# meenzen/Stl.Fusion

Hardware: AMD Instinct MI355X
Metric: invalidated nodes/sec + GTEPS at 1/2/4/8 MI355X; achieved HBM GB/s vs peak (higher is better)
Workload: dtype u64

## Files before the change

### include/fgi.h

```cpp
#ifndef FGI_H
#define FGI_H
#include <stddef.h>
#include <stdint.h>

#ifdef __cplusplus
extern "C" {
#endif

typedef int fgi_status;
#define FGI_OK 0
#define FGI_EINVAL 1
#define FGI_ENOMEM 2
#define FGI_ECAPACITY 3
#define FGI_EDEVICE 4
#define FGI_ESTATE 5
#define FGI_ENOTSUP 6

#define FGI_NONE 0xFFFFFFFFu

#define FGI_COMPUTING 0u
#define FGI_CONSISTENT 1u
#define FGI_INVALIDATED 2u
#define FGI_STATE_MASK 3u
#define FGI_F_INVALIDATE_ON_SET_OUTPUT 4u
// ... 158 lines not shown
fgi_status fgi_stream(fgi_graph* g, void** stream);
#define FGI_OPT_DEAD_FILTER 1
#define FGI_OPT_DIRECTION 2
#define FGI_OPT_PULL_ALPHA 3
#define FGI_OPT_LEVEL_TIMING 4
#define FGI_OPT_PULL_BETA 5
#define FGI_OPT_DEFRAG_PCT 6
#define FGI_OPT_PART_COLLECTIVES 7
#define FGI_OPT_PULL_TPB 8
#define FGI_OPT_FRONT_EXCHANGE 9
#define FGI_OPT_HOT_HEADS 10
#define FGI_OPT_FAULT_INJECT 11
#define FGI_OPT_PART_PLAN 13
#define FGI_OPT_PART_BUCKET 14
#define FGI_OPT_FAULT_INJECT_TAIL 16
fgi_status fgi_set_option(fgi_graph* g, int option, int64_t value);

fgi_status fgi_part_unique_id(uint8_t* id128);
fgi_status fgi_part_init(fgi_graph* g, uint32_t n_global, const uint8_t* id128);
typedef int (*fgi_allgather_fn)(void* ctx, const void* send, uint64_t bytes, void* recv);
fgi_status fgi_part_init_host(fgi_graph* g, uint32_t n_global, fgi_allgather_fn fn, void* ctx);
fgi_status fgi_part_synth_rmat(fgi_graph* g, uint32_t scale, uint32_t edge_factor, uint64_t seed,
                               uint32_t stale_pct, uint64_t stale_seed);
fgi_status fgi_part_register_nodes(fgi_graph* g, uint32_t n, const uint32_t* slot, const uint64_t* version,
                                   const uint32_t* state_flags);
fgi_status fgi_part_load_edges(fgi_graph* g, uint64_t m, const uint32_t* used, const uint32_t* dependant,
                               const uint64_t* tag);
fgi_status fgi_part_invalidate(fgi_graph* g, uint32_t n_roots, const uint32_t* roots_dev,
                               const uint8_t* immediately_dev, uint64_t* out_n, fgi_wave_stats* stats);
fgi_status fgi_part_export_ids(fgi_graph* g, uint32_t* out_ids, uint64_t cap, uint64_t* out_n);
// ... 27 lines not shown
```

### stl.fusion_amd/csrc/fgi_internal.h

```cpp
#pragma once
#include <hip/hip_runtime.h>
#include <stdint.h>

#include <chrono>
#include <cstdlib>
#include <string>
#include <utility>
#include <vector>

#include "../../include/fgi.h"
#include "../../include/fgi_variants.h"

#ifndef FGI_VARIANTS
#define FGI_VARIANTS 0
#endif

namespace fgi {

constexpr uint64_t kVMask = (1ull << 56) - 1;
constexpr int kStateShift = 56;
constexpr uint64_t kStateBits = 3ull << kStateShift;
constexpr uint64_t kW_IOSO = 1ull << 58;
constexpr uint64_t kW_DS = 1ull << 59;
constexpr uint64_t kW_HasDelay = 1ull << 60;
// ... 70 lines not shown
    *src = rmat_scramble(s, scale, seed);
    *dst = rmat_scramble(d, scale, seed);
}
__host__ __device__ inline bool synth_stale(uint32_t stale_pct, uint64_t stale_seed, uint32_t src, uint32_t dst) {
    return stale_pct && (sm64(stale_seed ^ sm64(((uint64_t)src << 32) | dst)) % 100) < stale_pct;
}

constexpr int kRing = 64;
constexpr int kBlock = 256;
constexpr int kEPT = 8;
constexpr int kChunk = kBlock * kEPT;
constexpr int kFine = 256;
constexpr uint32_t kStatBlocks = 8192;
constexpr int kStatCols = 8;
constexpr int kPullTile = 1024;
constexpr int kDoneGroups = 16;
constexpr int kDoneStride = 16;
#ifndef FGI_FINAL_BLOCKS
#define FGI_FINAL_BLOCKS 1024
#endif
#ifndef FGI_FINAL_WPB
#define FGI_FINAL_WPB 256
#endif
#ifndef FGI_INIT_BLOCKS
#define FGI_INIT_BLOCKS 2048
#endif
constexpr uint32_t kFinalBlocks = FGI_FINAL_BLOCKS;
constexpr uint32_t kFinalWpb = FGI_FINAL_WPB;
constexpr uint32_t kInitBlocks = FGI_INIT_BLOCKS;
#ifndef FGI_SPIN_WAIT
// ... 246 lines not shown
    std::vector<uint32_t> flg_drop;
    uint32_t* inv_bm = nullptr;
    uint64_t bm_words = 0;

    uint64_t* uin_off = nullptr;
    uint32_t* uin_len = nullptr;
    uint32_t* uin_src = nullptr;
    uint64_t* uin_head = nullptr;
    uint32_t* uin_more = nullptr;
    uint64_t uin_cap = 0;
    unsigned long long* pool_live = nullptr;
    uint64_t pool_live_cap = 0;
    uint64_t pl_mut_epoch = 0, pl_pool_epoch = ~0ull;
    uint4* cand = nullptr;
    uint32_t* cand_seg = nullptr;
    uint32_t* wl = nullptr;
    uint32_t* hot_id = nullptr;
    uint32_t n_hot = 0;
    uint64_t hot_w0 = 0;
    uint4* sv[2] = {nullptr, nullptr};
    uint32_t* sv_cnt[2] = {nullptr, nullptr};
    uint64_t cand_cap = 0;
    uint32_t cand_grid = 0;
    uint64_t uin_epoch = 0;
    uint64_t mut_epoch = 1;
    uint64_t epoch_counter = 1;
    uint64_t snap_mut_epoch = 0;

    int opt_dead_filter = 1;
    int opt_defrag_pct = 60;
    int opt_part_coll = 0;
    int opt_front_exchange = 0;
    uint64_t stale_est = 0;
    uint32_t prune_cursor = 0;
    int opt_direction = 0;
    int opt_pull_alpha = 28;
    int opt_pull_tpb = 0;
    int opt_hot_heads = 0;
    uint32_t* sum_bm = nullptr;
    int64_t opt_sum_min = -1;
    int opt_pull_beta = 32;
    int opt_level_timing = 1;
    int opt_fused = fgi::fused_default();

    void* scratch = nullptr;
    size_t scratch_bytes = 0;
    unsigned long long* misc_dev = nullptr;
    unsigned long long* misc_host = nullptr;

    uint64_t* snap_node = nullptr;
    uint64_t* snap_row_off = nullptr;
    uint32_t* snap_row_len = nullptr;
    uint32_t* snap_row_cap = nullptr;
// ... 184 lines not shown
```

### stl.fusion_amd/csrc/graph.hip

```cpp
#include <hip/hip_runtime.h>
#include <hip/hip_cooperative_groups.h>

#include <rocprim/device/device_radix_sort.hpp>
#include <rocprim/device/device_reduce.hpp>
#include <rocprim/device/device_segmented_radix_sort.hpp>
#include <rocprim/device/device_scan.hpp>

#include <algorithm>
#include <cstddef>
#include <chrono>
#include <cstdarg>
#include <cstdio>
#include <cstring>

#include "fgi_internal.h"

namespace fgi {

fgi_status set_err(fgi_graph* g, fgi_status st, const char* fmt, ...) {
    if (g) {
        char buf[512];
        va_list ap;
        va_start(ap, fmt);
        vsnprintf(buf, sizeof(buf), fmt, ap);
// ... 1056 lines not shown
    const uint64_t key = k < k_max ? sorted[k] : 0ull;
    if ((key >> 32) == 0) {
        hot_id[k] = FGI_NONE;
        return;
    }
    hot_id[k] = (uint32_t)key;
    hot_rank[(uint32_t)key] = k;
}

__device__ __forceinline__ uint32_t head_code(uint32_t h, const uint32_t* hot_rank, uint32_t hot_bit0) {
    if (h == FGI_NONE || !hot_rank) return h;
    const uint32_t r = hot_rank[h];
    return r != FGI_NONE ? (hot_bit0 + r) : h;
}

__global__ void k_cand_fill(uint32_t n, const uint32_t* __restrict__ flag, const uint32_t* __restrict__ pos,
                            const uint64_t* __restrict__ uin_head, const uint32_t* __restrict__ uin_len,
                            const uint32_t* __restrict__ row_len, const uint32_t* __restrict__ hot_rank,
                            uint32_t hot_bit0, uint4* cand, unsigned long long* too_long) {
    const uint32_t d = blockIdx.x * blockDim.x + threadIdx.x;
    if (d >= n || !flag[d]) return;
    const uint32_t p = pos[d], rl = row_len[d];
    if (rl >> 31) atomicAdd(too_long, 1ull);
    const uint64_t h = uin_head[d];
    cand[p] = make_uint4(d, (rl & 0x7FFFFFFFu) | (uin_len[d] > 2 ? 0x80000000u : 0u),
                         head_code((uint32_t)h, hot_rank, hot_bit0), head_code((uint32_t)(h >> 32), hot_rank, hot_bit0));
}

__global__ void k_cand_seg(uint32_t G, uint64_t span, uint32_t n, const uint32_t* __restrict__ pos, uint32_t total,
                           uint32_t* seg) {
    const uint32_t b = blockIdx.x * blockDim.x + threadIdx.x;
    if (b > G) return;
    const uint64_t s0 = (uint64_t)b * span;
    seg[b] = s0 < n ? pos[s0] : total;
}

__global__ void k_invalidate_all_roots(uint32_t n_slots, const unsigned long long* node, uint32_t* roots,
                                       unsigned long long* cnt) {
    const uint32_t s = blockIdx.x * blockDim.x + threadIdx.x;
    if (s < n_slots && word_is_current(node[s])) roots[atomicAdd(cnt, 1ull)] = s;
}

inline uint32_t nblk(uint64_t n, uint32_t b = 256) { return (uint32_t)((n + b - 1) / b); }

template <class T>
fgi_status h2d(fgi_graph* g, T* dst, const T* src, size_t count) {
    if (count == 0) return FGI_OK;
    FGI_HIP(g, hipMemcpyAsync(dst, src, count * sizeof(T), hipMemcpyHostToDevice, g->stream));
    return FGI_OK;
// ... 226 lines not shown
    if (G == 0) return FGI_OK;
    hipStream_t s = g->stream;
    const uint32_t N = g->n_slots;
    if (g->cand_cap < N || !g->cand) {
        dfree(g->cand);
        dfree(g->wl);
        for (int k = 0; k < 2; ++k) dfree(g->sv[k]);
        g->cand_cap = 0;
        FGI_TRY(dmalloc(g, &g->cand, N));
        FGI_TRY(dmalloc(g, &g->wl, N));
        for (int k = 0; k < 2; ++k) FGI_TRY(dmalloc(g, &g->sv[k], N));
        g->cand_cap = N;
    }
    if (!g->cand_seg) {
        FGI_TRY(dmalloc(g, &g->cand_seg, (size_t)kStatBlocks + 1));
        FGI_TRY(dmalloc(g, &g->sv_cnt[0], kStatBlocks));
        FGI_TRY(dmalloc(g, &g->sv_cnt[1], kStatBlocks));
    }
    Tmp tf, tp, ts;
    uint32_t *flag, *pos;
    FGI_TRY(tmalloc(g, tf, &flag, N));
    FGI_TRY(tmalloc(g, tp, &pos, N));
    hipLaunchKernelGGL(k_cand_flag, dim3(nblk(N)), dim3(256), 0, s, N, g->uin_len, flag);
    size_t tb = 0;
    FGI_HIP(g, rocprim::exclusive_scan(nullptr, tb, flag, pos, 0u, (size_t)N, rocprim::plus<uint32_t>(), s));
    char* tmp;
    FGI_TRY(tmalloc(g, ts, &tmp, tb));
    FGI_HIP(g, rocprim::exclusive_scan(tmp, tb, flag, pos, 0u, (size_t)N, rocprim::plus<uint32_t>(), s));
    uint32_t lp = 0, lf = 0;
    FGI_TRY(d2h(g, &lp, pos + N - 1, 1));
    FGI_TRY(d2h(g, &lf, flag + N - 1, 1));
    const uint32_t total = lp + lf;
    Tmp th;
    uint32_t* hot_rank = nullptr;
    g->n_hot = 0;
    PartView pv;
    const bool part = part_view(g, &pv);
    const uint32_t NH = part ? pv.n_global : g->n_handles;
    g->hot_w0 = part ? pv.front_words_global : g->bm_words;
    if (g->hot_w0 * 32 + kHot < (uint64_t)FGI_NONE) {
        if (!g->hot_id) FGI_TRY(dmalloc(g, &g->hot_id, kHot));
        Tmp tc, tk0, tk1, tt;
        uint32_t* cnt;
        uint64_t *k0, *k1;
        FGI_TRY(tmalloc(g, tc, &cnt, NH));
        FGI_TRY(tmalloc(g, th, &hot_rank, NH));
        FGI_TRY(tmalloc(g, tk0, &k0, NH));
// ... 5 lines not shown
        size_t sb = 0;
        FGI_HIP(g, rocprim::radix_sort_keys_desc(nullptr, sb, k0, k1, (size_t)NH, 0, 64, s));
        char* st;
        FGI_TRY(tmalloc(g, tt, &st, sb));
        FGI_HIP(g, rocprim::radix_sort_keys_desc(st, sb, k0, k1, (size_t)NH, 0, 64, s));
        uint32_t n_hot = hot_count(NH);
        if (g->opt_hot_heads > 0)
            n_hot = std::min<uint32_t>(n_hot, (uint32_t)(g->opt_hot_heads + 255) / 256 * 256);
        hipLaunchKernelGGL(k_hot_pick, dim3(n_hot / 256), dim3(256), 0, s, NH, n_hot, k1, g->hot_id, hot_rank);
        FGI_HIP(g, hipGetLastError());
        FGI_HIP(g, hipStreamSynchronize(s));
        g->n_hot = n_hot;
    }
    FGI_HIP(g, hipMemsetAsync(g->misc_dev + 15, 0, sizeof(unsigned long long), s));
    hipLaunchKernelGGL(k_cand_fill, dim3(nblk(N)), dim3(256), 0, s, N, flag, pos, g->uin_head, g->uin_len, g->row_len,
                       hot_rank, (uint32_t)(g->hot_w0 * 32), g->cand, g->misc_dev + 15);
    hipLaunchKernelGGL(k_cand_seg, dim3(nblk(G + 1)), dim3(256), 0, s, G, (uint64_t)tpb * kPullTile, N, pos, total,
                       g->cand_seg);
    FGI_HIP(g, hipGetLastError());
    unsigned long long too_long = 0;
    FGI_TRY(d2h(g, &too_long, g->misc_dev + 15, 1));
    if (too_long == 0) g->cand_grid = G;
    if (getenv("FGI_TRACE"))
        fprintf(stderr, "[fgi] candidates: %u of %u slots, pull grid %u x %u tiles, %u hot heads, %llu rows too long\n", total,
                N, G, tpb, g->n_hot, (unsigned long long)too_long);
    return FGI_OK;
}

fgi_status build_rows_from_keys(fgi_graph* g, uint64_t m, uint64_t* keys, uint64_t* tags, uint64_t ver_seed,
                                uint32_t stale_pct, uint64_t stale_seed, uint32_t src_base, uint32_t dst_base) {
    hipStream_t s = g->stream;
    const uint32_t H = g->n_handles;
    FGI_HIP(g, hipMemsetAsync(g->row_off, 0, (size_t)H * sizeof(uint64_t), s));
    FGI_HIP(g, hipMemsetAsync(g->row_len, 0, (size_t)H * sizeof(uint32_t), s));
    FGI_HIP(g, hipMemsetAsync(g->row_cap, 0, (size_t)H * sizeof(uint32_t), s));
    FGI_HIP(g, hipMemsetAsync(g->used_cnt, 0, (size_t)H * sizeof(uint32_t), s));
    g->pool_top = 0;
    g->pool_epoch++;
    touch(g);
    if (m == 0) return FGI_OK;
// ... 335 lines not shown
        dfree(g->fr_off[i]);
        dfree(g->fr_len[i]);
    }
    for (int i = 0; i < 2; ++i) {
        dfree(g->escan[i]);
        dfree(g->cstart[i]);
    }
    dfree(g->uin_off);
    dfree(g->uin_len);
    dfree(g->uin_src);
    dfree(g->uin_head);
    dfree(g->pool_live);
    dfree(g->cand);
    dfree(g->wl);
    dfree(g->cand_seg);
    dfree(g->hot_id);
    for (int k = 0; k < 2; ++k) {
        dfree(g->sv[k]);
        dfree(g->sv_cnt[k]);
    }
    dfree(g->vis_bm);
    dfree(g->vis_spare);
    if (g->flg_bm) (void)hipFree(g->flg_bm);
    if (g->flg_cnt) (void)hipFree(g->flg_cnt);
    for (int k = 0; k < 2; ++k)
        if (g->flg_out[k]) (void)hipFree(g->flg_out[k]);
    dfree(g->cls_bm);
    dfree(g->uin_more);
    dfree(g->sum_bm);
    dfree(g->inv_bm);
// ... 425 lines not shown
        return FGI_OK;
    case FGI_OPT_LEVEL_TIMING: g->opt_level_timing = value ? 1 : 0; return FGI_OK;
    case FGI_OPT_PULL_TPB:
        if (value < 0 || value > 32) return set_err(g, FGI_EINVAL, "pull tiles per block must be 0..32");
        g->opt_pull_tpb = (int)value;
        if (!g->part) {
            g->uin_epoch = 0;
        } else if (g->uin_src && g->uin_epoch == g->mut_epoch) {
            hipSetDevice(g->device);
            return build_candidates(g);
        }
        return FGI_OK;
    case FGI_OPT_HOT_HEADS:
        if (value < 0 || value > (int64_t)kHot) return set_err(g, FGI_EINVAL, "hot heads must be 0..%u", kHot);
        g->opt_hot_heads = (int)value;
        if (!g->part) {
            g->uin_epoch = 0;
        } else if (g->uin_src && g->uin_epoch == g->mut_epoch) {
            hipSetDevice(g->device);
            return build_candidates(g);
        }
        return FGI_OK;
    case FGI_OPT_PULL_BETA:
        if (value < 0) return set_err(g, FGI_EINVAL, "beta must be >= 0");
        g->opt_pull_beta = (int)value;
        return FGI_OK;
    case FGI_OPT_PART_PLAN: g->opt_part_plan = value ? 1 : 0; return FGI_OK;
    case FGI_OPT_PART_BUCKET: return part_set_bucket(g, value);
    case FGI_OPT_PROBE_SUMMARY:
        if (value < -1 || value > (int64_t)FGI_NONE) return set_err(g, FGI_EINVAL, "probe summary: -1 or a word count");
// ... 1527 lines not shown
```

### stl.fusion_amd/csrc/wave.hip

```cpp
#include <hip/hip_cooperative_groups.h>
#include <hip/hip_runtime.h>

#include <sched.h>

#include <algorithm>
#include <chrono>
#include <cstdio>
#include <cstring>
#include <cstdlib>
#include <vector>

#include "fgi_internal.h"

#ifndef FGI_PROBE
#define FGI_PROBE 0
#endif

namespace fgi {
namespace {

__device__ __forceinline__ uint32_t lane_id() { return __lane_id(); }
constexpr int kProbeLevelsOff = 1 << 20;

#if FGI_PROBE
// ... 834 lines not shown

struct PullArgs {
    uint32_t n_slots;
    const uint64_t* __restrict__ uin_off;
    const uint32_t* __restrict__ uin_len;
    const uint32_t* __restrict__ uin_src;
    const uint32_t* front_rd;
    const uint32_t* sum;
    uint32_t hot_bit0;
    uint32_t hot_lds;
    uint32_t* inv_bm;
    const uint32_t* __restrict__ cls;
    uint32_t* wl;
    unsigned long long* bsum;
    const uint32_t* __restrict__ cand_seg;
    const uint4* c[3];
    uint4* sv[2];
    uint32_t* sv_cnt[2];
};

constexpr uint32_t kMaxIter = 32;
#ifndef FGI_CPL
#define FGI_CPL 4
#endif
#ifndef FGI_TAIL_CAP
#define FGI_TAIL_CAP kChunk
#endif
constexpr uint32_t kCPL = FGI_CPL;
constexpr uint32_t kTailCap = FGI_TAIL_CAP;
constexpr uint32_t kTileWords = kPullTile / 64;
constexpr uint32_t kOwnWords = 2 * kMaxIter * kTileWords;
constexpr uint32_t kCandBatch = kCPL * kBlock;
constexpr uint32_t kWaveBatch = kCPL * 64;
constexpr uint32_t kWaveTailCap = kTailCap / (kBlock / 64);
constexpr uint32_t kLaneTail = 12;

struct PullLds {
    uint32_t hot[kLdsHot];
    uint32_t vm[kOwnWords];
    uint32_t wm[kOwnWords];
    uint32_t cs[kOwnWords];
    uint32_t sn;
    uint32_t wn;
};

constexpr uint32_t kPushLds = kChunkEmitCap + 8;
constexpr uint32_t kLevelLds =
    std::max<uint32_t>(kPushLds + (sizeof(MsgEmit<true>) + 7) / 8 * 2, kTailCap + 4 + (sizeof(PullLds) + 3) / 4);
static_assert(kTailCap % 4 == 0 && kWaveBatch <= kTailCap / (kBlock / 64), "pull tail queue");

// ... 5 lines not shown
typedef uint32_t u32x4 __attribute__((ext_vector_type(4)));

__device__ __forceinline__ bool sum_zero(const PullArgs& p, uint32_t h) {
    return !((p.sum[h >> 11] >> ((h >> 6) & 31)) & 1u);
}
__device__ __forceinline__ uint32_t head_bits(const PullArgs& p, const PullLds& s, uint32_t h, bool sum) {
    const uint32_t r = (h - p.hot_bit0) >> 5;
    if (r < p.hot_lds) return s.hot[r];
    if (sum && h < p.hot_bit0 && sum_zero(p, h)) return 0u;
    return p.front_rd[h >> 5];
}
__device__ __forceinline__ bool front_bit(const PullArgs& p, uint32_t u, bool sum) {
    return !(sum && sum_zero(p, u)) && bit_of(p.front_rd, u);
}

__device__ __forceinline__ uint4 load_cand(const uint4* p, bool in, uint32_t s_lo) {
    if (!in) return make_uint4(s_lo, 0u, FGI_NONE, FGI_NONE);
    const u32x4 v = __builtin_nontemporal_load(reinterpret_cast<const u32x4*>(p));
    return make_uint4(v.x, v.y, v.z, v.w);
}

__device__ __forceinline__ void pull_hit(const PullArgs& p, PullLds& s, uint64_t s_lo, uint64_t seg, uint32_t d, bool win,
                                         uint32_t aux, WinSum& ws) {
    const uint32_t rel = (uint32_t)(d - s_lo);
    const uint32_t bit = 1u << (d & 31);
    if (win) {
        atomicOr(&s.wm[rel >> 5], bit);
        const uint32_t rl = aux & 0x7FFFFFFFu;
        ++ws.w;
        if (rl) {
            ++ws.e;
            ws.l += rl;
            p.wl[seg + atomicAdd(&s.wn, 1u)] = d;
        }
    } else {
        atomicOr(&s.vm[rel >> 5], bit);
    }
}

__device__ __forceinline__ void pull_tails(const PullArgs& p, const uint4* src, uint4* sv_out, const unsigned long long* node,
                                           uint64_t s_lo, uint64_t seg, uint32_t* q, uint32_t nq, PullLds& s,
                                           uint32_t& flagged, uint32_t& examined, uint32_t& tails, WinSum& ws, bool sum) {
    const uint32_t lane = lane_id();
    uint32_t nlong = 0;
    for (uint32_t r0 = 0; r0 < nq; r0 += 64) {
        const uint32_t e = r0 + lane;
        const bool in = e < nq;
        uint32_t qi = 0, len = 0;
        uint64_t off = 0;
        uint4 c = make_uint4(0u, 0u, 0u, 0u);
        if (in) {
            qi = q[e];
            c = src[seg + qi];
            len = p.uin_len[c.x];
            off = p.uin_off[c.x];
        }
        const uint32_t u2 = (in && len > 2) ? p.uin_src[off + 2] : FGI_NONE;
        const uint32_t u3 = (in && len > 3) ? p.uin_src[off + 3] : FGI_NONE;
        const bool hit = (u2 != FGI_NONE && front_bit(p, u2, sum)) || (u3 != FGI_NONE && front_bit(p, u3, sum));
        examined += (u2 != FGI_NONE ? 1u : 0u) + (u3 != FGI_NONE ? 1u : 0u);
        const bool more = in && !hit && len > 4;
        const unsigned long long mm = __ballot(more);
        if (more) q[nlong + rank_in(mm)] = qi | (len > kLaneTail ? 0x80000000u : 0u);
        nlong += (uint32_t)__popcll(mm);
        if (in && hit) {
            const uint32_t d = c.x, rel = (uint32_t)(d - s_lo);
            const bool win = (s.cs[rel >> 5] >> (d & 31)) & 1u;
            pull_hit(p, s, s_lo, seg, d, win, c.y, ws);
            if (!win) flagged += first_visit(node[d]) == 2 ? 1u : 0u;
        }
        const bool surv = in && !hit && !more;
        const unsigned long long sm = __ballot(surv);
        if (sm) {
            uint32_t sb = 0;
            if (lane == 0) sb = atomicAdd(&s.sn, (uint32_t)__popcll(sm));
            sb = from_lane0(sb);
            if (surv) sv_out[sb + rank_in(sm)] = c;
        }
        tails += in ? 1u : 0u;
    }
    __builtin_amdgcn_wave_barrier();
    uint32_t nl2 = 0;
    for (uint32_t r0 = 0; r0 < nlong; r0 += 64) {
        const uint32_t e = r0 + lane;
        const uint32_t v = e < nlong ? q[e] : 0u;
        const bool in = e < nlong && !(v >> 31);
        const bool lng = e < nlong && (v >> 31);
        const unsigned long long lm = __ballot(lng);
        if (lng) q[nl2 + rank_in(lm)] = v & 0x7FFFFFFFu;
        nl2 += (uint32_t)__popcll(lm);
        uint4 c = make_uint4(0u, 0u, 0u, 0u);
        uint32_t len = 0;
        uint64_t off = 0;
        if (in) {
            c = src[seg + v];
            len = p.uin_len[c.x];
            off = p.uin_off[c.x];
        }
        uint32_t u[kLaneTail - 4];
#pragma unroll
        for (uint32_t k = 0; k < kLaneTail - 4; ++k) u[k] = (in && 4 + k < len) ? p.uin_src[off + 4 + k] : FGI_NONE;
        bool found = false;
#pragma unroll
        for (uint32_t k = 0; k < kLaneTail - 4; ++k)
            if (u[k] != FGI_NONE) {
                found |= front_bit(p, u[k], sum);
                ++examined;
            }
        if (in && found) {
            const uint32_t d = c.x, rel = (uint32_t)(d - s_lo);
            const bool win = (s.cs[rel >> 5] >> (d & 31)) & 1u;
            pull_hit(p, s, s_lo, seg, d, win, c.y, ws);
            if (!win) flagged += first_visit(node[d]) == 2 ? 1u : 0u;
        }
        const bool surv = in && !found;
        const unsigned long long sm = __ballot(surv);
        if (sm) {
            uint32_t sb = 0;
            if (lane == 0) sb = atomicAdd(&s.sn, (uint32_t)__popcll(sm));
            sb = from_lane0(sb);
            if (surv) sv_out[sb + rank_in(sm)] = c;
        }
    }
    nlong = nl2;
    __builtin_amdgcn_wave_barrier();
    const uint32_t sub = lane & 7, grp = lane >> 3;
    constexpr uint32_t G8 = 8;
    uint4 c_n = make_uint4(0u, 0u, 0u, 0u);
    uint32_t len_n = 0;
    uint64_t off_n = 0;
    if (grp < nlong) {
        c_n = src[seg + q[grp]];
        len_n = p.uin_len[c_n.x];
        off_n = p.uin_off[c_n.x];
    }
    for (uint32_t e = grp; e < nlong; e += G8) {
        const uint4 c = c_n;
        const uint32_t len = len_n;
        const uint64_t off = off_n;
        if (e + G8 < nlong) {
            c_n = src[seg + q[e + G8]];
            len_n = p.uin_len[c_n.x];
            off_n = p.uin_off[c_n.x];
        }
        bool found = false;
        for (uint32_t r = 4; r < len && !found; r += 8) {
            const uint32_t k = r + sub;
            const bool x = k < len && front_bit(p, p.uin_src[off + k], sum);
            examined += (k < len) ? 1u : 0u;
            found = ((__ballot(x) >> (lane & ~7u)) & 0xFFull) != 0;
        }
        if (sub == 0) {
            const uint32_t d = c.x;
            if (found) {
                const uint32_t rel = (uint32_t)(d - s_lo);
                const bool win = (s.cs[rel >> 5] >> (d & 31)) & 1u;
                pull_hit(p, s, s_lo, seg, d, win, c.y, ws);
                if (!win) flagged += first_visit(node[d]) == 2 ? 1u : 0u;
            } else {
                sv_out[atomicAdd(&s.sn, 1u)] = c;
            }
        }
    }
}

__device__ __forceinline__ void pull_level(int L, const PullArgs& p, const WaveParams& wp, uint64_t npull, bool sum,
                                           const unsigned long long* node, uint32_t* vis, uint32_t* lds_q, PullLds& s,
                                           unsigned long long* blk, unsigned long long (*s_st)[kStats],
                                           unsigned long long (&bs)[3]) {
    uint32_t flagged = 0, examined = 0, live = 0, tails = 0, examined_tail = 0;
    const uint32_t lane = lane_id();
    const uint32_t b = blockIdx.x;
    const uint64_t s_lo = (uint64_t)b * wp.tpb * kPullTile;
    const uint64_t seg = p.cand_seg[b];
    const int sid = npull == 0 ? 0 : 1 + (int)((npull - 1) & 1);
    const int dst = (int)(npull & 1);
    const uint4* src = p.c[sid];
    const uint32_t seg_n = (uint32_t)(p.cand_seg[b + 1] - seg);
    const uint32_t cnt = npull == 0 ? seg_n : min(p.sv_cnt[sid - 1][b], seg_n);
    uint4* const sv_out = p.sv[dst] + seg;
    uint32_t* const wl_out = p.wl + seg;
    uint4 c[kCPL];
#pragma unroll
    for (int j = 0; j < (int)kCPL; ++j) {
        const uint32_t i = (threadIdx.x >> 6) * kWaveBatch + j * 64 + lane;
        c[j] = load_cand(src + seg + i, i < cnt, (uint32_t)s_lo);
    }
    {
        const uint64_t w_lo = s_lo >> 5, w_end = ((uint64_t)p.n_slots + 31) >> 5;
        const uint32_t nw = 2 * wp.tpb * kTileWords;
        constexpr uint32_t kPer = kOwnWords / kBlock;
        constexpr uint32_t kHotPer = kLdsHot / kBlock;
        uint32_t vv[kPer], cc[kPer], hh[kHotPer];
#pragma unroll
        for (uint32_t k = 0; k < kPer; ++k) {
            const uint32_t i = threadIdx.x + k * kBlock;
            const bool in = i < nw && w_lo + i < w_end;
            vv[k] = in ? vis[w_lo + i] : ~0u;
            cc[k] = in ? p.cls[w_lo + i] : 0u;
        }
        const uint32_t* hot = p.front_rd + (p.hot_bit0 >> 5);
// ... 18 lines not shown
        s.sn = 0;
        s.wn = 0;
    }
    __syncthreads();
    PROBE(L, 1);
    WinSum ws;
    const uint32_t wid = threadIdx.x >> 6;
    uint32_t* wq = lds_q + wid * kWaveTailCap;
    uint32_t qn = 0;
    for (uint32_t base = wid * kWaveBatch; base < cnt; base += kCandBatch) {
        bool lv[kCPL];
        uint32_t f0[kCPL], f1[kCPL];
#pragma unroll
        for (int j = 0; j < (int)kCPL; ++j) {
            const bool in = base + j * 64 + lane < cnt;
            const uint32_t rel = c[j].x - (uint32_t)s_lo;
            lv[j] = in && !((s.vm[rel >> 5] >> (c[j].x & 31)) & 1u);
            f0[j] = lv[j] ? head_bits(p, s, c[j].z, sum) : 0u;
            f1[j] = (lv[j] && c[j].w != FGI_NONE) ? head_bits(p, s, c[j].w, sum) : 0u;
        }
        uint4 cn[kCPL];
#pragma unroll
        for (int j = 0; j < (int)kCPL; ++j) {
            const uint32_t i = base + kCandBatch + j * 64 + lane;
            cn[j] = load_cand(src + seg + i, i < cnt, (uint32_t)s_lo);
        }
#pragma unroll
        for (int j = 0; j < (int)kCPL; ++j) {
            const uint32_t i = base + j * 64 + lane;
            const uint32_t d = c[j].x, h0 = c[j].z, h1 = c[j].w, aux = c[j].y;
            const bool b0 = lv[j] && ((f0[j] >> (h0 & 31)) & 1u);
            const bool b1 = lv[j] && h1 != FGI_NONE && ((f1[j] >> (h1 & 31)) & 1u);
            const bool hit = b0 || b1;
            const bool tail = lv[j] && !hit && (aux >> 31);
            const bool surv = lv[j] && !hit && !tail;
            live += lv[j] ? 1u : 0u;
            examined += (lv[j] ? 1u : 0u) + ((lv[j] && h1 != FGI_NONE && !b0) ? 1u : 0u);
            bool win = false;
            if (hit) {
                const uint32_t rel = d - (uint32_t)s_lo;
                const uint32_t bit = 1u << (d & 31);
                win = (s.cs[rel >> 5] & bit) != 0;
                if (win) {
                    atomicOr(&s.wm[rel >> 5], bit);
                    const uint32_t rl = aux & 0x7FFFFFFFu;
                    ++ws.w;
                    ws.e += rl ? 1u : 0u;
                    ws.l += rl;
                } else {
                    atomicOr(&s.vm[rel >> 5], bit);
                    flagged += first_visit(node[d]) == 2 ? 1u : 0u;
                }
            }
            const bool xw = win && (aux & 0x7FFFFFFFu);
            const unsigned long long xm = __ballot(xw);
            if (xm) {
                uint32_t xb = 0;
                if (lane == 0) xb = atomicAdd(&s.wn, (uint32_t)__popcll(xm));
                xb = from_lane0(xb);
                if (xw) wl_out[xb + rank_in(xm)] = d;
            }
            const unsigned long long tm = __ballot(tail);
            if (tail) wq[qn + rank_in(tm)] = i;
            qn += (uint32_t)__popcll(tm);
            const unsigned long long sm = __ballot(surv);
            if (sm) {
                uint32_t sb = 0;
                if (lane == 0) sb = atomicAdd(&s.sn, (uint32_t)__popcll(sm));
                sb = from_lane0(sb);
                if (surv) sv_out[sb + rank_in(sm)] = c[j];
            }
        }
        if (base + kCandBatch >= cnt) PROBE(L, 7);
        if (qn > kWaveTailCap - kWaveBatch || base + kCandBatch >= cnt) {
            __builtin_amdgcn_wave_barrier();
            pull_tails(p, src, sv_out, node, s_lo, seg, wq, qn, s, flagged, examined_tail, tails, ws,
                       sum);
            __builtin_amdgcn_wave_barrier();
            qn = 0;
        }
#pragma unroll
        for (int j = 0; j < (int)kCPL; ++j) c[j] = cn[j];
    }
    PROBE(L, 2);
    __syncthreads();
    PROBE(L, 3);
    unsigned long long* vis64 = reinterpret_cast<unsigned long long*>(vis);
    unsigned long long* inv64 = reinterpret_cast<unsigned long long*>(p.inv_bm);
    for (uint32_t i = threadIdx.x; i < wp.tpb * kTileWords; i += blockDim.x) {
        const uint64_t sl = s_lo + (uint64_t)i * 64;
        if (sl < p.n_slots) {
// ... 1325 lines not shown
PullArgs pull_args(fgi_graph* g, uint32_t n_slots, const uint32_t* front_rd) {
    PullArgs p;
    p.n_slots = n_slots;
    p.uin_off = g->uin_off;
    p.uin_len = g->uin_len;
    p.uin_src = g->uin_src;
    p.front_rd = front_rd;
    p.sum = ((g->part != nullptr) == (front_rd != g->inv_bm)) ? g->sum_bm : nullptr;
    p.hot_bit0 = (uint32_t)(g->hot_w0 * 32);
    p.hot_lds = std::min<uint32_t>(g->n_hot / 32, kLdsHot);
    p.inv_bm = g->inv_bm;
    p.wl = g->wl;
    p.cls = g->cls_bm;
    p.bsum = g->bsum;
    p.cand_seg = g->cand_seg;
    p.c[0] = g->cand;
    for (int k = 0; k < 2; ++k) {
        p.c[1 + k] = g->sv[k];
        p.sv[k] = g->sv[k];
        p.sv_cnt[k] = g->sv_cnt[k];
    }
    return p;
}

ExpandArgs expand_args(fgi_graph* g, int buf) {
    static const uint64_t small_max = [] {
        const char* e = getenv("FGI_PUSH_SMALL");
        return e && *e ? (uint64_t)strtoull(e, nullptr, 10) : kPushSmallMax;
    }();
    ExpandArgs x{g->fr_off[buf], g->escan[buf], g->cstart[buf], g->pool_col, g->pool_tag, g->opt_dead_filter};
// ... 1345 lines not shown
```

### stl.fusion_amd/fgi.py

```python
from __future__ import annotations

import ctypes as C
import os
from typing import Optional, Tuple

import numpy as np

_HERE = os.path.dirname(os.path.abspath(__file__))
LIB_PATH = os.environ.get("FGI_LIBRARY") or os.path.join(_HERE, "lib", "libfgi.so")

OK, EINVAL, ENOMEM, ECAPACITY, EDEVICE, ESTATE, ENOTSUP = range(7)
OPT_DEAD_FILTER, OPT_DIRECTION, OPT_PULL_ALPHA, OPT_LEVEL_TIMING, OPT_PULL_BETA, OPT_DEFRAG_PCT = 1, 2, 3, 4, 5, 6
OPT_PART_COLLECTIVES = 7
OPT_PULL_TPB = 8
OPT_FRONT_EXCHANGE = 9
OPT_HOT_HEADS = 10
OPT_FAULT_INJECT = 11
OPT_FUSED = 12
OPT_PART_PLAN = 13
OPT_PART_BUCKET = 14
OPT_FAULT_INJECT_TAIL = 16
OPT_PROBE_SUMMARY = 15
DIR_AUTO, DIR_PUSH, DIR_PULL = 0, 1, 2
NONE = 0xFFFFFFFF
COMPUTING, CONSISTENT, INVALIDATED = 0, 1, 2
F_IOSO, F_DELAY_STARTED, F_HAS_DELAY = 4, 8, 16
USED_ADDED, USED_DROPPED, USED_INVALIDATED, USED_ESTATE = range(4)

_STATUS = {0: "FGI_OK", 1: "FGI_EINVAL", 2: "FGI_ENOMEM", 3: "FGI_ECAPACITY", 4: "FGI_EDEVICE",
           5: "FGI_ESTATE", 6: "FGI_ENOTSUP"}


class FgiError(RuntimeError):
    def __init__(self, status: int, msg: str):
        super().__init__(f"{_STATUS.get(status, status)}: {msg}")
        self.status = status

# ... 706 lines not shown
```

Baseline: 32.94 billion.

## Pack tail adjacency into per-segment contiguous runs and compact candidate records

Builds a dense tail-run array (trun) that copies each candidate's adjacency list beyond the first two heads, along with its length, into contiguous per-block storage addressed by a run offset packed into the candidate record. The candidate record now stores a block-relative slot, tail flag, row length and run offset instead of the absolute slot. The pull tail passes read this run directly rather than chasing uin_len/uin_off/uin_src, so the dependent gathers should coalesce better. In exchange it adds a scan, a fill kernel and extra memory at candidate-build time, plus a fallback path for offsets or lengths that overflow.

```diff
diff --git a/include/fgi.h b/include/fgi.h
--- a/include/fgi.h
+++ b/include/fgi.h
@@ -196,6 +196,7 @@
 #define FGI_OPT_PART_PLAN 13
 #define FGI_OPT_PART_BUCKET 14
 #define FGI_OPT_FAULT_INJECT_TAIL 16
+#define FGI_OPT_RUN_OFFSET_BITS 17
 fgi_status fgi_set_option(fgi_graph* g, int option, int64_t value);
 
 fgi_status fgi_part_unique_id(uint8_t* id128);
diff --git a/stl.fusion_amd/csrc/fgi_internal.h b/stl.fusion_amd/csrc/fgi_internal.h
--- a/stl.fusion_amd/csrc/fgi_internal.h
+++ b/stl.fusion_amd/csrc/fgi_internal.h
@@ -108,6 +108,26 @@
 constexpr uint32_t kStatBlocks = 8192;
 constexpr int kStatCols = 8;
 constexpr int kPullTile = 1024;
+constexpr uint32_t kRecSlotBits = 15;
+constexpr uint32_t kRecLenEsc = (1u << 20) - 1;
+constexpr uint32_t kRecOffBits = 28;
+constexpr uint32_t kRecNoOff = (1u << kRecOffBits) - 1;
+__host__ __device__ inline void rec_encode(uint32_t rel, bool tail, uint32_t row_len, uint64_t run_off, uint64_t off_limit,
+                                           uint32_t& x, uint32_t& y) {
+    const uint32_t rl = row_len < kRecLenEsc ? row_len : kRecLenEsc;
+    const uint32_t ro = (tail && run_off < off_limit && run_off < kRecNoOff) ? (uint32_t)run_off : kRecNoOff;
+    x = rel | (tail ? 1u << kRecSlotBits : 0u) | (rl << 16);
+    y = (rl >> 16) | (ro << 4);
+}
+struct CandRec {
+    uint32_t rel;
+    bool tail;
+    uint32_t row_len;
+    uint32_t run_off;
+};
+__host__ __device__ inline CandRec rec_decode(uint32_t x, uint32_t y) {
+    return CandRec{x & ((1u << kRecSlotBits) - 1), ((x >> kRecSlotBits) & 1u) != 0, (x >> 16) | ((y & 15u) << 16), y >> 4};
+}
 constexpr int kDoneGroups = 16;
 constexpr int kDoneStride = 16;
 #ifndef FGI_FINAL_BLOCKS
@@ -384,6 +404,9 @@
     uint64_t pl_mut_epoch = 0, pl_pool_epoch = ~0ull;
     uint4* cand = nullptr;
     uint32_t* cand_seg = nullptr;
+    uint32_t* trun = nullptr;
+    uint64_t trun_cap = 0;
+    uint64_t* run_seg = nullptr;
     uint32_t* wl = nullptr;
     uint32_t* hot_id = nullptr;
     uint32_t n_hot = 0;
@@ -407,6 +430,7 @@
     int opt_pull_alpha = 28;
     int opt_pull_tpb = 0;
     int opt_hot_heads = 0;
+    int opt_run_off_bits = (int)fgi::kRecOffBits;
     uint32_t* sum_bm = nullptr;
     int64_t opt_sum_min = -1;
     int opt_pull_beta = 32;
diff --git a/stl.fusion_amd/csrc/graph.hip b/stl.fusion_amd/csrc/graph.hip
--- a/stl.fusion_amd/csrc/graph.hip
+++ b/stl.fusion_amd/csrc/graph.hip
@@ -1094,25 +1094,58 @@
     return r != FGI_NONE ? (hot_bit0 + r) : h;
 }
 
+__global__ void k_run_words(uint32_t n, const uint32_t* __restrict__ uin_len, uint64_t* words) {
+    const uint32_t d = blockIdx.x * blockDim.x + threadIdx.x;
+    if (d < n) words[d] = uin_len[d] > 2 ? uin_len[d] - 1 : 0u;
+}
+
 __global__ void k_cand_fill(uint32_t n, const uint32_t* __restrict__ flag, const uint32_t* __restrict__ pos,
                             const uint64_t* __restrict__ uin_head, const uint32_t* __restrict__ uin_len,
                             const uint32_t* __restrict__ row_len, const uint32_t* __restrict__ hot_rank,
-                            uint32_t hot_bit0, uint4* cand, unsigned long long* too_long) {
+                            uint32_t hot_bit0, uint32_t span, const uint64_t* __restrict__ rpos, uint64_t off_limit,
+                            uint4* cand, unsigned long long* too_long) {
     const uint32_t d = blockIdx.x * blockDim.x + threadIdx.x;
     if (d >= n || !flag[d]) return;
     const uint32_t p = pos[d], rl = row_len[d];
     if (rl >> 31) atomicAdd(too_long, 1ull);
     const uint64_t h = uin_head[d];
-    cand[p] = make_uint4(d, (rl & 0x7FFFFFFFu) | (uin_len[d] > 2 ? 0x80000000u : 0u),
-                         head_code((uint32_t)h, hot_rank, hot_bit0), head_code((uint32_t)(h >> 32), hot_rank, hot_bit0));
+    const uint32_t rel = d % span;
+    uint32_t x, y;
+    rec_encode(rel, uin_len[d] > 2, rl, rpos[d] - rpos[d - rel], off_limit, x, y);
+    cand[p] = make_uint4(x, y, head_code((uint32_t)h, hot_rank, hot_bit0), head_code((uint32_t)(h >> 32), hot_rank, hot_bit0));
 }
 
 __global__ void k_cand_seg(uint32_t G, uint64_t span, uint32_t n, const uint32_t* __restrict__ pos, uint32_t total,
-                           uint32_t* seg) {
+                           const uint64_t* __restrict__ rpos, uint64_t run_total, uint32_t* seg, uint64_t* run_seg) {
     const uint32_t b = blockIdx.x * blockDim.x + threadIdx.x;
     if (b > G) return;
     const uint64_t s0 = (uint64_t)b * span;
     seg[b] = s0 < n ? pos[s0] : total;
+    run_seg[b] = s0 < n ? rpos[s0] : run_total;
+}
+
+constexpr uint32_t kRunOwn = 32;
+__global__ void k_run_fill(uint32_t n, const uint32_t* __restrict__ uin_len, const uint64_t* __restrict__ uin_off,
+                           const uint32_t* __restrict__ uin_src, const uint64_t* __restrict__ rpos, uint32_t* trun) {
+    const uint32_t d = blockIdx.x * blockDim.x + threadIdx.x;
+    const uint32_t len = d < n ? uin_len[d] : 0u;
+    unsigned long long off = 0, ro = 0;
+    if (len > 2) {
+        off = uin_off[d];
+        ro = rpos[d];
+        trun[ro] = len;
+    }
+    const uint32_t own = len > 2 ? (len < kRunOwn ? len : kRunOwn) : 0u;
+    for (uint32_t k = 2; k < own; ++k) trun[ro + k - 1] = uin_src[off + k];
+    unsigned long long m = __ballot(len > kRunOwn);
+    const uint32_t lane = threadIdx.x & 63;
+    while (m) {
+        const int l = __ffsll(m) - 1;
+        m &= m - 1;
+        const uint32_t ln = __shfl(len, l);
+        const unsigned long long o_s = __shfl(off, l), o_r = __shfl(ro, l);
+        for (uint32_t k = kRunOwn + lane; k < ln; k += 64) trun[o_r + k - 1] = uin_src[o_s + k];
+    }
 }
 
 __global__ void k_invalidate_all_roots(uint32_t n_slots, const unsigned long long* node, uint32_t* roots,
@@ -1369,6 +1402,7 @@
     }
     if (!g->cand_seg) {
         FGI_TRY(dmalloc(g, &g->cand_seg, (size_t)kStatBlocks + 1));
+        FGI_TRY(dmalloc(g, &g->run_seg, (size_t)kStatBlocks + 1));
         FGI_TRY(dmalloc(g, &g->sv_cnt[0], kStatBlocks));
         FGI_TRY(dmalloc(g, &g->sv_cnt[1], kStatBlocks));
     }
@@ -1386,6 +1420,29 @@
     FGI_TRY(d2h(g, &lp, pos + N - 1, 1));
     FGI_TRY(d2h(g, &lf, flag + N - 1, 1));
     const uint32_t total = lp + lf;
+    Tmp tw, tr, trs;
+    uint64_t *rwords, *rpos;
+    FGI_TRY(tmalloc(g, tw, &rwords, N));
+    FGI_TRY(tmalloc(g, tr, &rpos, N));
+    hipLaunchKernelGGL(k_run_words, dim3(nblk(N)), dim3(256), 0, s, N, g->uin_len, rwords);
+    size_t rb = 0;
+    FGI_HIP(g, rocprim::exclusive_scan(nullptr, rb, rwords, rpos, (uint64_t)0, (size_t)N, rocprim::plus<uint64_t>(), s));
+    char* rtmp;
+    FGI_TRY(tmalloc(g, trs, &rtmp, rb));
+    FGI_HIP(g, rocprim::exclusive_scan(rtmp, rb, rwords, rpos, (uint64_t)0, (size_t)N, rocprim::plus<uint64_t>(), s));
+    uint64_t rlp = 0, rlw = 0;
+    FGI_TRY(d2h(g, &rlp, rpos + N - 1, 1));
+    FGI_TRY(d2h(g, &rlw, rwords + N - 1, 1));
+    const uint64_t run_total = rlp + rlw;
+    if (g->trun_cap < run_total || !g->trun) {
+        dfree(g->trun);
+        g->trun = nullptr;
+        g->trun_cap = 0;
+        const uint64_t cap = std::max<uint64_t>(run_total, 1024);
+        FGI_TRY(dmalloc(g, &g->trun, cap + 2));
+        g->trun_cap = cap;
+    }
+    hipLaunchKernelGGL(k_run_fill, dim3(nblk(N)), dim3(256), 0, s, N, g->uin_len, g->uin_off, g->uin_src, rpos, g->trun);
     Tmp th;
     uint32_t* hot_rank = nullptr;
     g->n_hot = 0;
@@ -1421,16 +1478,18 @@
     }
     FGI_HIP(g, hipMemsetAsync(g->misc_dev + 15, 0, sizeof(unsigned long long), s));
     hipLaunchKernelGGL(k_cand_fill, dim3(nblk(N)), dim3(256), 0, s, N, flag, pos, g->uin_head, g->uin_len, g->row_len,
-                       hot_rank, (uint32_t)(g->hot_w0 * 32), g->cand, g->misc_dev + 15);
-    hipLaunchKernelGGL(k_cand_seg, dim3(nblk(G + 1)), dim3(256), 0, s, G, (uint64_t)tpb * kPullTile, N, pos, total,
-                       g->cand_seg);
+                       hot_rank, (uint32_t)(g->hot_w0 * 32), tpb * (uint32_t)kPullTile, rpos,
+                       (uint64_t)1 << g->opt_run_off_bits, g->cand, g->misc_dev + 15);
+    hipLaunchKernelGGL(k_cand_seg, dim3(nblk(G + 1)), dim3(256), 0, s, G, (uint64_t)tpb * kPullTile, N, pos, total, rpos,
+                       run_total, g->cand_seg, g->run_seg);
     FGI_HIP(g, hipGetLastError());
     unsigned long long too_long = 0;
     FGI_TRY(d2h(g, &too_long, g->misc_dev + 15, 1));
     if (too_long == 0) g->cand_grid = G;
     if (getenv("FGI_TRACE"))
-        fprintf(stderr, "[fgi] candidates: %u of %u slots, pull grid %u x %u tiles, %u hot heads, %llu rows too long\n", total,
-                N, G, tpb, g->n_hot, (unsigned long long)too_long);
+        fprintf(stderr,
+                "[fgi] candidates: %u of %u slots, pull grid %u x %u tiles, %u hot heads, %llu rows too long, %llu tail-run words\n",
+                total, N, G, tpb, g->n_hot, (unsigned long long)too_long, (unsigned long long)run_total);
     return FGI_OK;
 }
 
@@ -1796,6 +1855,8 @@
     dfree(g->cand);
     dfree(g->wl);
     dfree(g->cand_seg);
+    dfree(g->run_seg);
+    dfree(g->trun);
     dfree(g->hot_id);
     for (int k = 0; k < 2; ++k) {
         dfree(g->sv[k]);
@@ -2251,6 +2312,16 @@
     case FGI_OPT_HOT_HEADS:
         if (value < 0 || value > (int64_t)kHot) return set_err(g, FGI_EINVAL, "hot heads must be 0..%u", kHot);
         g->opt_hot_heads = (int)value;
+        if (!g->part) {
+            g->uin_epoch = 0;
+        } else if (g->uin_src && g->uin_epoch == g->mut_epoch) {
+            hipSetDevice(g->device);
+            return build_candidates(g);
+        }
+        return FGI_OK;
+    case FGI_OPT_RUN_OFFSET_BITS:
+        if (value < 1 || value > (int64_t)kRecOffBits) return set_err(g, FGI_EINVAL, "run offset bits must be 1..%u", kRecOffBits);
+        g->opt_run_off_bits = (int)value;
         if (!g->part) {
             g->uin_epoch = 0;
         } else if (g->uin_src && g->uin_epoch == g->mut_epoch) {
diff --git a/stl.fusion_amd/csrc/wave.hip b/stl.fusion_amd/csrc/wave.hip
--- a/stl.fusion_amd/csrc/wave.hip
+++ b/stl.fusion_amd/csrc/wave.hip
@@ -872,6 +872,9 @@
     uint32_t* wl;
     unsigned long long* bsum;
     const uint32_t* __restrict__ cand_seg;
+    const uint32_t* __restrict__ trun;
+    const uint64_t* __restrict__ run_seg;
+    const uint32_t* __restrict__ row_len;
     const uint4* c[3];
     uint4* sv[2];
     uint32_t* sv_cnt[2];
@@ -892,6 +895,8 @@
 constexpr uint32_t kWaveBatch = kCPL * 64;
 constexpr uint32_t kWaveTailCap = kTailCap / (kBlock / 64);
 constexpr uint32_t kLaneTail = 12;
+static_assert(kMaxIter * kPullTile <= (1u << kRecSlotBits), "a candidate's record holds a block-relative slot");
+static_assert(kLaneTail < (1u << 15), "pass 2a's queue entry holds the list length above the candidate index");
 
 struct PullLds {
     uint32_t hot[kLdsHot];
@@ -927,61 +932,82 @@
     return !(sum && sum_zero(p, u)) && bit_of(p.front_rd, u);
 }
 
-__device__ __forceinline__ uint4 load_cand(const uint4* p, bool in, uint32_t s_lo) {
-    if (!in) return make_uint4(s_lo, 0u, FGI_NONE, FGI_NONE);
+__device__ __forceinline__ uint4 load_cand(const uint4* p, bool in) {
+    if (!in) return make_uint4(0u, 0u, FGI_NONE, FGI_NONE);
     const u32x4 v = __builtin_nontemporal_load(reinterpret_cast<const u32x4*>(p));
     return make_uint4(v.x, v.y, v.z, v.w);
 }
 
-__device__ __forceinline__ void pull_hit(const PullArgs& p, PullLds& s, uint64_t s_lo, uint64_t seg, uint32_t d, bool win,
-                                         uint32_t aux, WinSum& ws) {
-    const uint32_t rel = (uint32_t)(d - s_lo);
-    const uint32_t bit = 1u << (d & 31);
+__device__ __forceinline__ uint32_t cand_row_len(const PullArgs& p, uint32_t d, const uint4& c) {
+    const uint32_t rl = rec_decode(c.x, c.y).row_len;
+    return rl == kRecLenEsc ? p.row_len[d] : rl;
+}
+
+__device__ __forceinline__ const uint32_t* list_at(const PullArgs& p, const uint32_t* run, uint32_t s_lo, const uint4& c,
+                                                   uint32_t& len) {
+    const uint32_t ro = rec_decode(c.x, c.y).run_off;
+    if (ro != kRecNoOff) {
+        len = run[ro];
+        return run + ro;
+    }
+    const uint32_t d = s_lo + rec_decode(c.x, c.y).rel;
+    len = p.uin_len[d];
+    return p.uin_src + p.uin_off[d] + 1;
+}
+
+__device__ __forceinline__ bool pull_hit(const PullArgs& p, PullLds& s, uint32_t s_lo, uint64_t seg, const uint4& c,
+                                         const unsigned long long* node, WinSum& ws) {
+    const uint32_t rel = rec_decode(c.x, c.y).rel, d = s_lo + rel;
+    const uint32_t bit = 1u << (rel & 31);
+    const bool win = (s.cs[rel >> 5] & bit) != 0;
     if (win) {
         atomicOr(&s.wm[rel >> 5], bit);
-        const uint32_t rl = aux & 0x7FFFFFFFu;
+        const uint32_t rl = cand_row_len(p, d, c);
         ++ws.w;
         if (rl) {
             ++ws.e;
             ws.l += rl;
             p.wl[seg + atomicAdd(&s.wn, 1u)] = d;
         }
-    } else {
-        atomicOr(&s.vm[rel >> 5], bit);
-    }
+        return false;
+    }
+    atomicOr(&s.vm[rel >> 5], bit);
+    return first_visit(node[d]) == 2;
 }
 
 __device__ __forceinline__ void pull_tails(const PullArgs& p, const uint4* src, uint4* sv_out, const unsigned long long* node,
-                                           uint64_t s_lo, uint64_t seg, uint32_t* q, uint32_t nq, PullLds& s,
-                                           uint32_t& flagged, uint32_t& examined, uint32_t& tails, WinSum& ws, bool sum) {
+                                           uint32_t s_lo, uint64_t seg, const uint32_t* run, uint32_t* q, uint32_t nq,
+                                           PullLds& s, uint32_t& flagged, uint32_t& examined, uint32_t& tails, WinSum& ws,
+                                           bool sum) {
     const uint32_t lane = lane_id();
     uint32_t nlong = 0;
     for (uint32_t r0 = 0; r0 < nq; r0 += 64) {
         const uint32_t e = r0 + lane;
         const bool in = e < nq;
-        uint32_t qi = 0, len = 0;
-        uint64_t off = 0;
+        uint32_t qi = 0, len = 0, u2 = FGI_NONE, u3 = FGI_NONE;
         uint4 c = make_uint4(0u, 0u, 0u, 0u);
         if (in) {
             qi = q[e];
             c = src[seg + qi];
-            len = p.uin_len[c.x];
-            off = p.uin_off[c.x];
-        }
-        const uint32_t u2 = (in && len > 2) ? p.uin_src[off + 2] : FGI_NONE;
-        const uint32_t u3 = (in && len > 3) ? p.uin_src[off + 3] : FGI_NONE;
+            const uint32_t ro = rec_decode(c.x, c.y).run_off;
+            if (ro != kRecNoOff) {
+                len = run[ro];
+                u2 = run[ro + 1];
+                const uint32_t t3 = run[ro + 2];
+                u3 = len > 3 ? t3 : FGI_NONE;
+            } else {
+                const uint32_t* lp = list_at(p, run, s_lo, c, len);
+                u2 = lp[1];
+                if (len > 3) u3 = lp[2];
+            }
+        }
         const bool hit = (u2 != FGI_NONE && front_bit(p, u2, sum)) || (u3 != FGI_NONE && front_bit(p, u3, sum));
         examined += (u2 != FGI_NONE ? 1u : 0u) + (u3 != FGI_NONE ? 1u : 0u);
         const bool more = in && !hit && len > 4;
         const unsigned long long mm = __ballot(more);
-        if (more) q[nlong + rank_in(mm)] = qi | (len > kLaneTail ? 0x80000000u : 0u);
+        if (more) q[nlong + rank_in(mm)] = qi | (len > kLaneTail ? 0x80000000u : len << 16);
         nlong += (uint32_t)__popcll(mm);
-        if (in && hit) {
-            const uint32_t d = c.x, rel = (uint32_t)(d - s_lo);
-            const bool win = (s.cs[rel >> 5] >> (d & 31)) & 1u;
-            pull_hit(p, s, s_lo, seg, d, win, c.y, ws);
-            if (!win) flagged += first_visit(node[d]) == 2 ? 1u : 0u;
-        }
+        if (in && hit) flagged += pull_hit(p, s, s_lo, seg, c, node, ws) ? 1u : 0u;
         const bool surv = in && !hit && !more;
         const unsigned long long sm = __ballot(surv);
         if (sm) {
@@ -1004,15 +1030,15 @@
         nl2 += (uint32_t)__popcll(lm);
         uint4 c = make_uint4(0u, 0u, 0u, 0u);
         uint32_t len = 0;
-        uint64_t off = 0;
+        const uint32_t* lp = nullptr;
         if (in) {
-            c = src[seg + v];
-            len = p.uin_len[c.x];
-            off = p.uin_off[c.x];
+            c = src[seg + (v & 0xFFFFu)];
+            lp = list_at(p, run, s_lo, c, len);
+            len = v >> 16;
         }
         uint32_t u[kLaneTail - 4];
 #pragma unroll
-        for (uint32_t k = 0; k < kLaneTail - 4; ++k) u[k] = (in && 4 + k < len) ? p.uin_src[off + 4 + k] : FGI_NONE;
+        for (uint32_t k = 0; k < kLaneTail - 4; ++k) u[k] = (in && 4 + k < len) ? lp[3 + k] : FGI_NONE;
         bool found = false;
 #pragma unroll
         for (uint32_t k = 0; k < kLaneTail - 4; ++k)
@@ -1020,12 +1046,7 @@
                 found |= front_bit(p, u[k], sum);
                 ++examined;
             }
-        if (in && found) {
-            const uint32_t d = c.x, rel = (uint32_t)(d - s_lo);
-            const bool win = (s.cs[rel >> 5] >> (d & 31)) & 1u;
-            pull_hit(p, s, s_lo, seg, d, win, c.y, ws);
-            if (!win) flagged += first_visit(node[d]) == 2 ? 1u : 0u;
-        }
+        if (in && found) flagged += pull_hit(p, s, s_lo, seg, c, node, ws) ? 1u : 0u;
         const bool surv = in && !found;
         const unsigned long long sm = __ballot(surv);
         if (sm) {
@@ -1041,35 +1062,29 @@
     constexpr uint32_t G8 = 8;
     uint4 c_n = make_uint4(0u, 0u, 0u, 0u);
     uint32_t len_n = 0;
-    uint64_t off_n = 0;
+    const uint32_t* lp_n = nullptr;
     if (grp < nlong) {
         c_n = src[seg + q[grp]];
-        len_n = p.uin_len[c_n.x];
-        off_n = p.uin_off[c_n.x];
+        lp_n = list_at(p, run, s_lo, c_n, len_n);
     }
     for (uint32_t e = grp; e < nlong; e += G8) {
         const uint4 c = c_n;
         const uint32_t len = len_n;
-        const uint64_t off = off_n;
+        const uint32_t* lp = lp_n;
         if (e + G8 < nlong) {
             c_n = src[seg + q[e + G8]];
-            len_n = p.uin_len[c_n.x];
-            off_n = p.uin_off[c_n.x];
+            lp_n = list_at(p, run, s_lo, c_n, len_n);
         }
         bool found = false;
         for (uint32_t r = 4; r < len && !found; r += 8) {
             const uint32_t k = r + sub;
-            const bool x = k < len && front_bit(p, p.uin_src[off + k], sum);
+            const bool x = k < len && front_bit(p, lp[k - 1], sum);
             examined += (k < len) ? 1u : 0u;
             found = ((__ballot(x) >> (lane & ~7u)) & 0xFFull) != 0;
         }
         if (sub == 0) {
-            const uint32_t d = c.x;
             if (found) {
-                const uint32_t rel = (uint32_t)(d - s_lo);
-                const bool win = (s.cs[rel >> 5] >> (d & 31)) & 1u;
-                pull_hit(p, s, s_lo, seg, d, win, c.y, ws);
-                if (!win) flagged += first_visit(node[d]) == 2 ? 1u : 0u;
+                flagged += pull_hit(p, s, s_lo, seg, c, node, ws) ? 1u : 0u;
             } else {
                 sv_out[atomicAdd(&s.sn, 1u)] = c;
             }
@@ -1093,11 +1108,12 @@
     const uint32_t cnt = npull == 0 ? seg_n : min(p.sv_cnt[sid - 1][b], seg_n);
     uint4* const sv_out = p.sv[dst] + seg;
     uint32_t* const wl_out = p.wl + seg;
+    const uint32_t* const run = p.trun + p.run_seg[b];
     uint4 c[kCPL];
 #pragma unroll
     for (int j = 0; j < (int)kCPL; ++j) {
         const uint32_t i = (threadIdx.x >> 6) * kWaveBatch + j * 64 + lane;
-        c[j] = load_cand(src + seg + i, i < cnt, (uint32_t)s_lo);
+        c[j] = load_cand(src + seg + i, i < cnt);
     }
     {
         const uint64_t w_lo = s_lo >> 5, w_end = ((uint64_t)p.n_slots + 31) >> 5;
@@ -1146,8 +1162,8 @@
 #pragma unroll
         for (int j = 0; j < (int)kCPL; ++j) {
             const bool in = base + j * 64 + lane < cnt;
-            const uint32_t rel = c[j].x - (uint32_t)s_lo;
-            lv[j] = in && !((s.vm[rel >> 5] >> (c[j].x & 31)) & 1u);
+            const uint32_t rel = rec_decode(c[j].x, c[j].y).rel;
+            lv[j] = in && !((s.vm[rel >> 5] >> (rel & 31)) & 1u);
             f0[j] = lv[j] ? head_bits(p, s, c[j].z, sum) : 0u;
             f1[j] = (lv[j] && c[j].w != FGI_NONE) ? head_bits(p, s, c[j].w, sum) : 0u;
         }
@@ -1155,27 +1171,27 @@
 #pragma unroll
         for (int j = 0; j < (int)kCPL; ++j) {
             const uint32_t i = base + kCandBatch + j * 64 + lane;
-            cn[j] = load_cand(src + seg + i, i < cnt, (uint32_t)s_lo);
+            cn[j] = load_cand(src + seg + i, i < cnt);
         }
 #pragma unroll
         for (int j = 0; j < (int)kCPL; ++j) {
             const uint32_t i = base + j * 64 + lane;
-            const uint32_t d = c[j].x, h0 = c[j].z, h1 = c[j].w, aux = c[j].y;
+            const uint32_t rel = rec_decode(c[j].x, c[j].y).rel, d = (uint32_t)s_lo + rel, h0 = c[j].z, h1 = c[j].w;
             const bool b0 = lv[j] && ((f0[j] >> (h0 & 31)) & 1u);
             const bool b1 = lv[j] && h1 != FGI_NONE && ((f1[j] >> (h1 & 31)) & 1u);
             const bool hit = b0 || b1;
-            const bool tail = lv[j] && !hit && (aux >> 31);
+            const bool tail = lv[j] && !hit && rec_decode(c[j].x, c[j].y).tail;
             const bool surv = lv[j] && !hit && !tail;
             live += lv[j] ? 1u : 0u;
             examined += (lv[j] ? 1u : 0u) + ((lv[j] && h1 != FGI_NONE && !b0) ? 1u : 0u);
             bool win = false;
+            uint32_t rl = 0;
             if (hit) {
-                const uint32_t rel = d - (uint32_t)s_lo;
-                const uint32_t bit = 1u << (d & 31);
+                const uint32_t bit = 1u << (rel & 31);
                 win = (s.cs[rel >> 5] & bit) != 0;
                 if (win) {
                     atomicOr(&s.wm[rel >> 5], bit);
-                    const uint32_t rl = aux & 0x7FFFFFFFu;
+                    rl = cand_row_len(p, d, c[j]);
                     ++ws.w;
                     ws.e += rl ? 1u : 0u;
                     ws.l += rl;
@@ -1184,7 +1200,7 @@
                     flagged += first_visit(node[d]) == 2 ? 1u : 0u;
                 }
             }
-            const bool xw = win && (aux & 0x7FFFFFFFu);
+            const bool xw = win && rl;
             const unsigned long long xm = __ballot(xw);
             if (xm) {
                 uint32_t xb = 0;
@@ -1206,7 +1222,7 @@
         if (base + kCandBatch >= cnt) PROBE(L, 7);
         if (qn > kWaveTailCap - kWaveBatch || base + kCandBatch >= cnt) {
             __builtin_amdgcn_wave_barrier();
-            pull_tails(p, src, sv_out, node, s_lo, seg, wq, qn, s, flagged, examined_tail, tails, ws,
+            pull_tails(p, src, sv_out, node, (uint32_t)s_lo, seg, run, wq, qn, s, flagged, examined_tail, tails, ws,
                        sum);
             __builtin_amdgcn_wave_barrier();
             qn = 0;
@@ -2562,6 +2578,9 @@
     p.cls = g->cls_bm;
     p.bsum = g->bsum;
     p.cand_seg = g->cand_seg;
+    p.trun = g->trun;
+    p.run_seg = g->run_seg;
+    p.row_len = g->row_len;
     p.c[0] = g->cand;
     for (int k = 0; k < 2; ++k) {
         p.c[1 + k] = g->sv[k];
diff --git a/stl.fusion_amd/fgi.py b/stl.fusion_amd/fgi.py
--- a/stl.fusion_amd/fgi.py
+++ b/stl.fusion_amd/fgi.py
@@ -21,6 +21,7 @@
 OPT_PART_BUCKET = 14
 OPT_FAULT_INJECT_TAIL = 16
 OPT_PROBE_SUMMARY = 15
+OPT_RUN_OFFSET_BITS = 17
 DIR_AUTO, DIR_PUSH, DIR_PULL = 0, 1, 2
 NONE = 0xFFFFFFFF
 COMPUTING, CONSISTENT, INVALIDATED = 0, 1, 2
```

Measured after the change: 34.33 billion (median of 6 runs). 4.2% higher.
